# sayands/sgaligner

Hardware: AMD Instinct MI355X
Metric: subscan-pairs/sec (fwd+bwd) + node-match Hits@1 vs reference (higher is better)
Workload: dtype f32 (fp32 operands and fp32 accumulation throughout; the anchors x negatives loss sweeps multiply them as three exact bf16 planes, six bf16 MFMAs per product...

## Files before the change

sgaligner_amd/csrc/sweep3.hip:

```cpp
#include <type_traits>

#include "loss_math.h"

namespace {

typedef __bf16 bf16x8 __attribute__((ext_vector_type(8)));
typedef __bf16 bf16x2 __attribute__((ext_vector_type(2)));
typedef float f32x2 __attribute__((ext_vector_type(2)));
typedef unsigned int u32x4 __attribute__((ext_vector_type(4)));
typedef unsigned int u32x2 __attribute__((ext_vector_type(2)));
typedef short s16x4 __attribute__((ext_vector_type(4)));

constexpr int S3_DP = 104;
constexpr int S3_PLANE = 3 * 2 * 1024;
constexpr int S3_TAIL = 3 * S3_PLANE;
constexpr int S3_BLOCK = S3_TAIL + 2048;
constexpr int S3_NCH = S3_BLOCK / 1024;
constexpr int S3_ROWSLOTS = 3 * 12 + 4;

__device__ __forceinline__ void split3_pair(float v0, float v1, unsigned& h, unsigned& m, unsigned& l) {
    const bf16x2 H = __builtin_convertvector(f32x2{v0, v1}, bf16x2);
    const unsigned hu = __builtin_bit_cast(unsigned, H);
#ifdef S3_SPLIT_DOT2
    unsigned c0 = 0x0000BF80u, c1 = 0xBF800000u;
    asm("" : "+s"(c0), "+s"(c1));
    const bf16x2 n0 = __builtin_bit_cast(bf16x2, c0), n1 = __builtin_bit_cast(bf16x2, c1);
    const float r0 = __builtin_amdgcn_fdot2_f32_bf16(H, n0, v0, false);
    const float r1 = __builtin_amdgcn_fdot2_f32_bf16(H, n1, v1, false);
#else
    const float r0 = v0 - __builtin_bit_cast(float, hu << 16);
    const float r1 = v1 - __builtin_bit_cast(float, hu & 0xffff0000u);
#endif
    const bf16x2 Mi = __builtin_convertvector(f32x2{r0, r1}, bf16x2);
    const unsigned mu = __builtin_bit_cast(unsigned, Mi);
#ifdef S3_SPLIT_DOT2
    const float s0 = __builtin_amdgcn_fdot2_f32_bf16(Mi, n0, r0, false);
    const float s1 = __builtin_amdgcn_fdot2_f32_bf16(Mi, n1, r1, false);
#else
    const float s0 = r0 - __builtin_bit_cast(float, mu << 16);
    const float s1 = r1 - __builtin_bit_cast(float, mu & 0xffff0000u);
#endif
    const bf16x2 Lo = __builtin_convertvector(f32x2{s0, s1}, bf16x2);
    h = hu; m = mu; l = __builtin_bit_cast(unsigned, Lo);
}
__device__ __forceinline__ f32x4 mfma_b(u32x4 a, u32x4 b, f32x4 c) {
    return __builtin_amdgcn_mfma_f32_16x16x32_bf16(__builtin_bit_cast(bf16x8, a), __builtin_bit_cast(bf16x8, b), c, 0, 0, 0);
}
__device__ __forceinline__ u32x2 tr_read16(const unsigned char* p) {
    return __builtin_bit_cast(u32x2, __builtin_amdgcn_ds_read_tr16_b64_v4i16((__attribute__((address_space(3))) s16x4*)(p)));
}
__device__ __forceinline__ unsigned long long sreg64(unsigned long long v) {
    const unsigned lo = __builtin_amdgcn_readfirstlane((unsigned)v), hi = __builtin_amdgcn_readfirstlane((unsigned)(v >> 32));
    return ((unsigned long long)hi << 32) | lo;
}
template <int X, int END, int NR, bool VALU_ALL> __device__ __forceinline__ void sgb_seq() {
    if constexpr (X < END) {
        __builtin_amdgcn_sched_group_barrier(0x008, 1, 0);
        if constexpr (X < NR) __builtin_amdgcn_sched_group_barrier(0x100, 1, 0);
        if constexpr (VALU_ALL || X < 2) __builtin_amdgcn_sched_group_barrier(0x002, 2, 0);
        sgb_seq<X + 1, END, NR, VALU_ALL>();
    }
}
__host__ __device__ constexpr int s3_slot(int g, int i) { return 16 * g + (i ^ (12 * (g & 1))); }

struct TLayout { int nbA, nb1, nb2; };
__host__ __device__ inline TLayout make_tlayout(int A, int J1, int J2) { return TLayout{(A + 31) / 32, (J1 + 31) / 32, (J2 + 31) / 32}; }

constexpr int S3_STAT_BYTES = 2048;
constexpr int S3_DREAL = 100;

constexpr int S3_CS_BLOCKS = 256;
__global__ __launch_bounds__(128) void split3_colsum_kernel(const float* __restrict__ Z, int R, double* __restrict__ part) {
    const int c = threadIdx.x;
    const int per = (R + gridDim.x - 1) / gridDim.x, r0 = blockIdx.x * per, r1 = min(R, r0 + per);
    if (c >= S3_DP) return;
    double acc = 0.0;
    for (int r = r0; r < r1; ++r) acc += (double)Z[(size_t)r * S3_DP + c];
    part[(size_t)blockIdx.x * S3_DP + c] = acc;
}
__global__ __launch_bounds__(128) void split3_stats_kernel(const double* __restrict__ part, int nblocks, int R, float* __restrict__ stat) {
    __shared__ double sq[128];
    const int c = threadIdx.x;
    double cs = 0.0;
    if (c < S3_DP) for (int b = 0; b < nblocks; ++b) cs += part[(size_t)b * S3_DP + c];
    float zb = (c < S3_DREAL && R > 0) ? (float)(cs / (double)R) : 0.f;
    sq[c] = (double)zb * (double)zb;
    __syncthreads();
    __shared__ double tot;
    if (c == 0) {
        double t = 0.0;
        for (int i = 0; i < 128; ++i) t += sq[i];
        tot = t;
    }
    __syncthreads();
    const bool centre = tot >= 0.25;
    if (!centre) zb = 0.f;
    if (c < S3_DP) stat[c] = zb;
    if (c == 0) { stat[S3_DP] = centre ? (float)(0.5 * tot) : 0.f; stat[S3_DP + 1] = centre ? 1.f : 0.f; }
}

__global__ __launch_bounds__(256) void split3_tables_kernel(const float* __restrict__ Z, int A, int J1, int J2, unsigned char* __restrict__ Zb,
                                                            const float* __restrict__ stat, float* __restrict__ Zc) {
    __shared__ float tile[32 * S3_DP];
    __shared__ float zbar[S3_DP];
    const TLayout L = make_tlayout(A, J1, J2);
    int b = blockIdx.x, old0, len;
    if (b < L.nbA) { old0 = 0; len = A; }
    else if (b < 2 * L.nbA) { b -= L.nbA; old0 = A; len = A; }
    else if (b < 2 * L.nbA + L.nb1) { b -= 2 * L.nbA; old0 = 2 * A; len = J1; }
    else { b -= 2 * L.nbA + L.nb1; old0 = 2 * A + J1; len = J2; }
    const int nvalid = min(32, len - 32 * b);
    const float* src = Z + (size_t)(old0 + 32 * b) * S3_DP;
    if (threadIdx.x < S3_DP) zbar[threadIdx.x] = stat[threadIdx.x];
    __syncthreads();
    for (int e = threadIdx.x; e < 32 * S3_DP; e += 256) {
        const int r = e / S3_DP, c = e - r * S3_DP;
        tile[e] = (r < nvalid && c < S3_DREAL) ? src[e] - zbar[c] : 0.f;
        if (Zc && old0 < 2 * A && r < nvalid) Zc[(size_t)(old0 + 32 * b) * S3_DP + e] = c == S3_DREAL + 1 ? 1.f : tile[e];
    }
    __syncthreads();
    if (threadIdx.x < 32) {
        const int r = threadIdx.x;
        if (r < nvalid) {
            double a = 0.0;
            for (int c = 0; c < S3_DREAL; ++c) a += (double)zbar[c] * (double)tile[r * S3_DP + c];
            tile[r * S3_DP + S3_DREAL] = (float)(a + (double)stat[S3_DP]);
            tile[r * S3_DP + S3_DREAL + 1] = 1.f;
        }
    }
    __syncthreads();
    unsigned* out = reinterpret_cast<unsigned*>(Zb + (size_t)blockIdx.x * S3_BLOCK);
    for (int e = threadIdx.x; e < 3 * 2 * 64 * 4; e += 256) {
        const int p = e & 3, st = (e >> 2) & 63, jh = (e >> 8) & 1, q = e >> 9;
        const int g = st >> 4, i = (st & 15) ^ (12 * (g & 1));
        const int row = 8 * (i >> 2) + 4 * jh + (i & 3), col = 32 * q + 8 * g + 2 * p;
        unsigned h, m, l;
        split3_pair(tile[row * S3_DP + col], tile[row * S3_DP + col + 1], h, m, l);
        out[e] = h; out[S3_PLANE / 4 + e] = m; out[2 * S3_PLANE / 4 + e] = l;
    }
    for (int e = threadIdx.x; e < 2 * 64 * 4; e += 256) {
        const int p = e & 3, st = (e >> 2) & 63, jh = (e >> 8) & 1;
        const int g = st >> 4, i = (st & 15) ^ (12 * (g & 1));
        const int row = 8 * (i >> 2) + 4 * jh + (i & 3), col = 96 + 2 * p;
        unsigned h, m, l;
        split3_pair(tile[row * S3_DP + col], tile[row * S3_DP + col + 1], h, m, l);
        out[S3_TAIL / 4 + e] = g < 2 ? h : (g == 2 ? m : l);
    }
}


__global__ __launch_bounds__(256) void centre_tables_kernel(const float* __restrict__ Z, int R, const float* __restrict__ stat, float* __restrict__ Zc) {
    const int lane = threadIdx.x & 63, wpb = blockDim.x >> 6;
    for (int r = blockIdx.x * wpb + (threadIdx.x >> 6); r < R; r += gridDim.x * wpb) {
        const float* z = Z + (size_t)r * S3_DP;
        float* o = Zc + (size_t)r * S3_DP;
        double acc = 0.0;
        float v[2];
#pragma unroll
        for (int t = 0; t < 2; ++t) {
            const int d = lane + 64 * t;
            const float zb = d < S3_DREAL ? stat[d] : 0.f;
            v[t] = d < S3_DREAL ? z[d] - zb : 0.f;
            acc += (double)zb * (double)v[t];
        }
        acc = wave_sum_d(acc);
        o[lane] = v[0];
        const int d1 = lane + 64;
        if (d1 < S3_DP) o[d1] = d1 < S3_DREAL ? v[1] : (d1 == S3_DREAL ? (float)(acc + (double)stat[S3_DP]) : (d1 == S3_DREAL + 1 ? 1.f : 0.f));
    }
}

#ifdef S3_DBG_TIMING
__device__ unsigned long long g_s3_dbg[16];
#define S3_T(i) { const unsigned long long t_ = __builtin_readcyclecounter(); tacc[i] += t_ - tprev; tprev = t_; }
#else
#define S3_T(i)
#endif
struct TSeg { int blk0, jt_lo, jt_hi, old0, lo, hi, fam; };
struct TGroup { int own0, nown, own_old0, own_blk0, blk0, nsplit, nseg; TSeg seg[2]; };
struct TArgs {
    int M; const unsigned char* Zb[4]; int perm[4]; int ngroups; TGroup grp[4];
    float k0, k1, it0, it1, ka;
    const float* beta;
    double* sums;
    const double* gs;
    float* dZ[4];
    double* gamma;
};

template <int M, bool GRAD, int WV, int MG, bool GAM, bool LITE, bool FOLD>
__device__ __forceinline__ void sweep3_body(const TArgs& a, const int g) {
    static_assert(!LITE || !GRAD, "LITE: the forward sums only");
    static_assert(!FOLD || (GRAD && WV == 4), "FOLD: the one-wave-per-SIMD gradient sweep only");
    constexpr int NCT = 7;
    constexpr int WAVES = WV, THREADS = WAVES * 64;
    constexpr int OWN = WV * 16;
    constexpr int NCH = LITE ? S3_NCH - S3_PLANE / 1024 : S3_NCH;
    constexpr int KMAX = (NCH + WAVES - 1) / WAVES;
    constexpr int BUF = M * S3_BLOCK;
    constexpr bool PIPE = WV == 4;
#ifndef S3_OWN_IN_S
#define S3_OWN_IN_S 1
#endif
    constexpr bool OWN_IN_S = GRAD && PIPE && S3_OWN_IN_S;
#ifndef S3_SPREAD
#define S3_SPREAD 1
#endif
    constexpr bool SPREAD = OWN_IN_S && S3_SPREAD && !FOLD;
    extern __shared__ __attribute__((aligned(16))) unsigned char lds3[];

    const int tid = threadIdx.x, lane = tid & 63, wave = tid >> 6, g4 = lane >> 4, l15 = lane & 15;
    const TGroup& grp = a.grp[g];
    const int wg_in_grp = (int)blockIdx.x - grp.blk0;
    const int nsplit = grp.nsplit, n_ob = (grp.nown + OWN - 1) / OWN, n_units = n_ob * nsplit;
    const int unit = (wg_in_grp & 7) * ((n_units + 7) >> 3) + (wg_in_grp >> 3);
    if ((wg_in_grp >> 3) >= ((n_units + 7) >> 3) || unit >= n_units) return;
    const int split = unit / n_ob;
    const int own0 = grp.own0 + (unit - split * n_ob) * OWN;
    const int own_end = grp.own0 + grp.nown;
    const int wrow0 = own0 + wave * 16;
#ifdef S3_DBG_TIMING
    unsigned long long tacc[8] = {0, 0, 0, 0, 0, 0, 0, 0}, tprev = __builtin_readcyclecounter();
#endif

    u32x4 opl[M][3][3], otl[M][2];
    float beta[M];
    const bool iv = wrow0 + l15 < own_end;
    {
        const int my_i = wrow0 + l15;
        const int rel = (iv ? my_i : own0) - grp.own_old0;
        const int o = rel & 31, oi = 4 * (o >> 3) + (o & 3), ojh = (o >> 2) & 1;
        const size_t off = (size_t)(grp.own_blk0 + (rel >> 5)) * S3_BLOCK;
#pragma unroll
        for (int m = 0; m < M; ++m) {
            const unsigned char* base = a.Zb[m] + off;
#pragma unroll
            for (int p = 0; p < 3; ++p)
#pragma unroll
                for (int q = 0; q < 3; ++q) {
                    const int so = ((q * 2 + ojh) * 64 + s3_slot(g4, oi)) * 16;
                    opl[m][p][q] = iv ? *reinterpret_cast<const u32x4*>(base + p * S3_PLANE + so) : u32x4{0, 0, 0, 0};
                }
            u32x4 th = iv ? *reinterpret_cast<const u32x4*>(base + S3_TAIL + (ojh * 64 + s3_slot(0, oi)) * 16) : u32x4{0, 0, 0, 0};
            u32x4 tm = iv ? *reinterpret_cast<const u32x4*>(base + S3_TAIL + (ojh * 64 + s3_slot(2, oi)) * 16) : u32x4{0, 0, 0, 0};
            u32x4 tl = iv ? *reinterpret_cast<const u32x4*>(base + S3_TAIL + (ojh * 64 + s3_slot(3, oi)) * 16) : u32x4{0, 0, 0, 0};
            const float ksc = a.k1;
            auto rescale = [&](u32x4& ph, u32x4& pm, u32x4& pl) {
#pragma unroll
                for (int d = 0; d < 4; ++d) {
                    const float x0 = (__builtin_bit_cast(float, ph[d] << 16) + __builtin_bit_cast(float, pm[d] << 16)) + __builtin_bit_cast(float, pl[d] << 16);
                    const float x1 = (__builtin_bit_cast(float, ph[d] & 0xffff0000u) + __builtin_bit_cast(float, pm[d] & 0xffff0000u)) + __builtin_bit_cast(float, pl[d] & 0xffff0000u);
                    unsigned nh, nm, nl;
                    split3_pair(x0 * ksc, x1 * ksc, nh, nm, nl);
                    ph[d] = nh; pm[d] = nm; pl[d] = nl;
                }
            };
#pragma unroll
            for (int q = 0; q < 3; ++q) rescale(opl[m][0][q], opl[m][1][q], opl[m][2][q]);
            rescale(th, tm, tl);
            otl[m][0] = g4 == 1 ? tm : th;
            otl[m][1] = g4 == 0 ? tl : (g4 == 2 ? tm : u32x4{0, 0, 0, 0});
#pragma unroll
            for (int t = 0; t < 2; ++t)
                otl[m][t][2] = (otl[m][t][2] >> 16) | (otl[m][t][2] << 16);
        }
    }
#pragma unroll
    for (int m = 0; m < M; ++m) beta[m] = a.beta[a.perm[m]];

    constexpr int NSM = GRAD ? (FOLD ? 1 : MG) : 1;
    f32x4 gacc[GRAD ? MG : 1][NCT], gsm[NSM][NCT];
#pragma unroll
    for (int m = 0; m < (GRAD ? MG : 1); ++m)
#pragma unroll
        for (int ct = 0; ct < NCT; ++ct) gacc[m][ct] = f32x4{0.f, 0.f, 0.f, 0.f};
#pragma unroll
    for (int m = 0; m < NSM; ++m)
#pragma unroll
        for (int ct = 0; ct < NCT; ++ct) gsm[m][ct] = f32x4{0.f, 0.f, 0.f, 0.f};
    float gam[M];
#pragma unroll
    for (int m = 0; m < M; ++m) gam[m] = 0.f;

    const int wave_u = __builtin_amdgcn_readfirstlane(wave);
    const unsigned l16 = (threadIdx.x & 63u) * 16u;
    __amdgpu_buffer_rsrc_t rs[M];
    typedef __attribute__((address_space(3))) unsigned char* lds_ptr;
    constexpr bool LAST_ODD = KMAX * WAVES > NCH || (LITE && KMAX * WAVES > 2 * (S3_PLANE / 1024));
    unsigned crot[M], clast[M], trot[M], brot[M];
    unsigned tile_off = 0, buf_off = 0;
#pragma unroll
    for (int m = 0; m < M; ++m) {
        const int rot = (wave_u + m) & (WAVES - 1);
        int c = rot + (KMAX - 1) * WAVES;
        c = c >= NCH ? c - WAVES : c;
        if (LITE) c = c >= 2 * (S3_PLANE / 1024) ? c + S3_PLANE / 1024 : c;
        crot[m] = (unsigned)rot * 1024u; clast[m] = (unsigned)c * 1024u;
        trot[m] = 0; brot[m] = 0;
    }
    auto set_seg = [&](const TSeg& sgm) {
#pragma unroll
        for (int m = 0; m < M; ++m)
            rs[m] = __builtin_amdgcn_make_buffer_rsrc(const_cast<unsigned char*>(a.Zb[m]) + (size_t)sgm.blk0 * S3_BLOCK, (short)0,
                                                      (int)((unsigned)sgm.jt_hi * (unsigned)S3_BLOCK), 0x00020000);
    };
    auto set_tile = [&](int jt, unsigned char* buf) {
        tile_off = (unsigned)jt * (unsigned)S3_BLOCK;
        buf_off = (unsigned)(buf - lds3);
#pragma unroll
        for (int m = 0; m < M; ++m) {
            trot[m] = tile_off + crot[m]; brot[m] = buf_off + (unsigned)(m * S3_BLOCK) + crot[m];
            asm("" : "+s"(trot[m]), "+s"(brot[m]));
        }
    };
    auto issue_slots = [&](int f_lo, int f_hi) {
#ifdef S3_DBG_NODMA
        return;
#endif
#ifdef S3_DBG_DMA_WAVES
        unsigned dma_mask = S3_DBG_DMA_WAVES;
        asm volatile("" : "+s"(dma_mask));
        if (!((dma_mask >> wave_u) & 1u)) return;
#endif
#pragma unroll
        for (int f = f_lo; f < f_hi; ++f) {
            if (f >= M * KMAX) break;
            const int m = f / KMAX, k = f % KMAX;
            unsigned so, lo;
            if (LAST_ODD && k == KMAX - 1) { so = tile_off + clast[m]; lo = buf_off + (unsigned)(m * S3_BLOCK) + clast[m]; }
            else { so = trot[m] + (unsigned)(k * WAVES * 1024); lo = brot[m] + (unsigned)(k * WAVES * 1024); }
            __builtin_amdgcn_raw_ptr_buffer_load_lds(rs[m], (lds_ptr)lds3 + lo, 16, l16, so, 0, 0);
        }
    };
    auto issue = [&](int jt, unsigned char* buf) { set_tile(jt, buf); issue_slots(0, M * KMAX); };

    const int aoff = s3_slot(g4, l15) * 16;
    const int tr_io = 4 * g4 + (l15 >> 2), tr_cs = l15 & 3;
    const int tr_main = s3_slot(tr_cs >> 1, tr_io) * 16 + (tr_cs & 1) * 8;
    const int tr_tail = S3_TAIL + tr_io * 16 + (tr_cs & 1) * 8;
    const int tr_tail_l = S3_TAIL + (48 + (tr_io ^ 12)) * 16 + (tr_cs & 1) * 8;

#pragma unroll 1
    for (int sg = 0; sg < 2; ++sg) {
        if (sg >= grp.nseg) break;
        const TSeg seg = grp.seg[sg];
        set_seg(seg);
        float c0[M + 1], c1[M + 1];
#pragma unroll
        for (int m = 0; m <= M; ++m) {
            const int mo = m < M ? a.perm[m] : M;
            c0[m] = GRAD ? (float)(a.gs[mo * 8 + seg.fam * 2 + 0] * (double)a.it0) : 0.f;
            c1[m] = GRAD ? (float)(a.gs[mo * 8 + seg.fam * 2 + 1] * (double)a.it1) : 0.f;
        }
        const float ka = a.ka;
        double dsum[M + 1][2];
#pragma unroll
        for (int m = 0; m <= M; ++m) { dsum[m][0] = 0.0; dsum[m][1] = 0.0; }
        float pl0[LITE ? M + 1 : 1], pl1[LITE ? M + 1 : 1];
#pragma unroll
        for (int m = 0; m < (LITE ? M + 1 : 1); ++m) { pl0[m] = 0.f; pl1[m] = 0.f; }

        __syncthreads();
        if (seg.jt_lo + split < seg.jt_hi) issue(seg.jt_lo + split, lds3);
        int it = 0;
#pragma unroll 1
        for (int jt = seg.jt_lo + split; jt < seg.jt_hi; jt += nsplit, ++it) {
            unsigned char* buf = lds3 + (it & 1) * BUF;
            const int j0 = seg.old0 + 32 * jt;
            S3_T(5)
            __syncthreads();
            S3_T(0)
            const int next_jt = jt + nsplit < seg.jt_hi ? jt + nsplit : jt;
            unsigned char* next_buf = lds3 + ((it + 1) & 1) * BUF;
            set_tile(next_jt, next_buf);
            S3_T(1)
            if (GRAD) {
                const int vlo = max(seg.lo - j0, 0), vhi = min(seg.hi - j0, 32);
                if (vlo > 0 || vhi < 32) {
                    for (int x = tid; x < M * 32 * S3_ROWSLOTS; x += THREADS) {
                        const int pc = x % S3_ROWSLOTS, w = (x / S3_ROWSLOTS) % 32, m = x / (S3_ROWSLOTS * 32);
                        if (w >= vlo && w < vhi) continue;
                        const int wjh = (w >> 2) & 1, wi = 4 * (w >> 3) + (w & 3);
                        unsigned char* base = buf + m * S3_BLOCK;
                        if (pc < 36) {
                            const int pl = pc / 12, q = (pc % 12) >> 2, gq = pc & 3;
                            *reinterpret_cast<u32x4*>(base + pl * S3_PLANE + ((q * 2 + wjh) * 64 + s3_slot(gq, wi)) * 16) = u32x4{0, 0, 0, 0};
                        } else {
                            const int gq = pc - 36;
                            *reinterpret_cast<u32x4*>(base + S3_TAIL + (wjh * 64 + s3_slot(gq, wi)) * 16) = u32x4{0, 0, 0, 0};
                        }
                    }
                    __syncthreads();
                }
            }

            f32x4 sacc[M][2];
            float own[M][2][4];
            float cj[2][4];
            auto substep_wait = [&](int ss) {
                if (ss > 0) { __builtin_amdgcn_s_waitcnt(0xc07f); __builtin_amdgcn_sched_barrier(0); }
            };
            constexpr int NSET = PIPE ? 2 : 1;
            u32x4 at[NSET], ap[NSET][3][3];
            auto ld_one = [&](int ss, int idx) {
                const int e = ss % NSET;
                const unsigned char* ar = buf + (SPREAD ? ss % M : ss >> 1) * S3_BLOCK + (SPREAD ? ss / M : ss & 1) * 1024 + aoff;
                if (idx < 1) at[e] = *reinterpret_cast<const u32x4*>(ar + S3_TAIL);
                else ap[e][2 - (idx - 1) / 3][(idx - 1) % 3] = *reinterpret_cast<const u32x4*>(ar + (2 - (idx - 1) / 3) * S3_PLANE + ((idx - 1) % 3) * 2048);
            };
            auto ld_set = [&](int ss) {
#pragma unroll
                for (int idx = 0; idx < 10; ++idx) if (!(LITE && idx >= 1 && idx <= 3)) ld_one(ss, idx);
            };
            if (PIPE) {
                ld_set(0);
                __builtin_amdgcn_s_waitcnt(0xc07f);
                __builtin_amdgcn_sched_barrier(0);
            }
            if constexpr (SPREAD) {
                constexpr int NDS = 2 * M - 2, PER = (M * KMAX + NDS - 1) / NDS;
                constexpr int PA[6] = {2, 1, 1, 0, 0, 0}, PB[6] = {0, 1, 0, 2, 1, 0};
                f32x4 accp[2][2];
                float ot0 = 0.f, ot1 = 0.f, sjt = 0.f, ce0 = 0.f, ce1 = 0.f;
                auto own_step = [&](int mm, int hh, int r, int k) {
                    const float sv = sacc[mm][hh][r];
                    if (k == 0) ot0 = fexp2(sv * ka);
                    else if (k == 1) ot1 = fexp2(sv);
                    else own[mm][hh][r] = fmaf(c0[mm], ot0, c1[mm] * ot1);
                };
                auto cj_step = [&](int hh, int r, int k) {
                    if (k == 0) {
                        sjt = 0.f;
#pragma unroll
                        for (int mm = 0; mm < M; ++mm) sjt = fmaf(beta[mm], sacc[mm][hh][r], sjt);
                    } else if (k == 1) ce0 = fexp2(sjt * ka);
                    else if (k == 2) ce1 = fexp2(sjt);
                    else cj[hh][r] = c0[M] * ce0 + c1[M] * ce1;
                };
#pragma unroll
                for (int ss = 0; ss < 2 * M; ++ss) {
                    const int m = ss % M, jh = ss / M, e = ss % NSET, pa = ss & 1;
                    const int pm = ss > 0 ? (ss - 1) % M : 0, pjh = ss > 0 ? (ss - 1) / M : 0;
                    accp[pa][0] = f32x4{0.f, 0.f, 0.f, 0.f}; accp[pa][1] = f32x4{0.f, 0.f, 0.f, 0.f};
                    substep_wait(ss);
#pragma unroll
                    for (int x = 0; x < 20; ++x) {
                        if (x == 0) accp[pa][0] = mfma_b(at[e], otl[m][1], accp[pa][0]);
                        else if (x == 1) accp[pa][1] = mfma_b(at[e], otl[m][0], accp[pa][1]);
                        else accp[pa][x & 1] = mfma_b(ap[e][PA[(x - 2) / 3]][(x - 2) % 3], opl[m][PB[(x - 2) / 3]][(x - 2) % 3], accp[pa][x & 1]);
                        __builtin_amdgcn_sched_barrier(0);
                        if (ss + 1 < 2 * M && x < 10) ld_one(ss + 1, x);
                        if (ss < NDS && (x % 3) == 1 && (x / 3) < PER) issue_slots(ss * PER + (x / 3), ss * PER + (x / 3) + 1);
                        if (ss > 0) {
                            if (x == 0) { sacc[pm][pjh][0] = accp[pa ^ 1][0][0] + accp[pa ^ 1][1][0]; sacc[pm][pjh][1] = accp[pa ^ 1][0][1] + accp[pa ^ 1][1][1]; }
                            if (x == 2) { sacc[pm][pjh][2] = accp[pa ^ 1][0][2] + accp[pa ^ 1][1][2]; sacc[pm][pjh][3] = accp[pa ^ 1][0][3] + accp[pa ^ 1][1][3]; }
                            if (pm < MG) {
                                constexpr int G0[4] = {3, 8, 12, 16}, G1[4] = {5, 9, 14, 17}, G2[4] = {6, 11, 15, 18};
#pragma unroll
                                for (int r = 0; r < 4; ++r) {
                                    if (x == G0[r]) own_step(pm, pjh, r, 0);
                                    if (x == G1[r]) own_step(pm, pjh, r, 1);
                                    if (x == G2[r]) own_step(pm, pjh, r, 2);
                                }
                            }
                        }
                        if (ss >= NDS) {
                            const int q = (x == 19 ? 5 : (x % 3) == 1 && x <= 13 ? x / 3 : -1);
                            if (q >= 0) {
                                const int qq = (ss - NDS) * 6 + q, r = qq / 3, k = qq % 3;
                                if (k == 0) { if (r > 0) cj_step(0, r - 1, 3); cj_step(0, r, 0); }
                                else cj_step(0, r, k);
                            }
                        }
                        __builtin_amdgcn_sched_barrier(0);
                    }
                }
#pragma unroll
                for (int r = 0; r < 4; ++r) sacc[M - 1][1][r] = accp[(2 * M - 1) & 1][0][r] + accp[(2 * M - 1) & 1][1][r];
                cj_step(0, 3, 3);
            } else {
#pragma unroll
            for (int ss = 0; ss < 2 * M; ++ss) {
                const int m = ss >> 1, jh = ss & 1, e = ss % NSET;
                if (!PIPE) ld_set(ss);
                if (PIPE) substep_wait(ss);
                constexpr int NDS = GRAD ? (2 * M - 2) : 2 * M, PER = (M * KMAX + NDS - 1) / NDS;
                f32x4 acc2[2] = {f32x4{0.f, 0.f, 0.f, 0.f}, f32x4{0.f, 0.f, 0.f, 0.f}};
                float ownt[2] = {0.f, 0.f};
                constexpr int PA[6] = {2, 1, 1, 0, 0, 0}, PB[6] = {0, 1, 0, 2, 1, 0};
#pragma unroll
                for (int x = 0; x < 20; ++x) {
                    const bool skip = LITE && x >= 2 && (PA[(x - 2) / 3] == 2 || PB[(x - 2) / 3] == 2 || (PA[(x - 2) / 3] == 1 && PB[(x - 2) / 3] == 1));
                    if (skip) {}
                    else if (x == 0) acc2[0] = mfma_b(at[e], otl[m][1], acc2[0]);
                    else if (x == 1) acc2[1] = mfma_b(at[e], otl[m][0], acc2[1]);
                    else acc2[x & 1] = mfma_b(ap[e][PA[(x - 2) / 3]][(x - 2) % 3], opl[m][PB[(x - 2) / 3]][(x - 2) % 3], acc2[x & 1]);
                    if (PIPE) {
                        __builtin_amdgcn_sched_barrier(0);
                        if (ss + 1 < 2 * M && x < 10 && !(LITE && x >= 1 && x <= 3)) ld_one(ss + 1, x);
                        if (ss < NDS && (x % 3) == 1 && (x / 3) < PER) issue_slots(ss * PER + (x / 3), ss * PER + (x / 3) + 1);
                        if (OWN_IN_S && m > 0 && m - 1 < MG && x >= 11 && x < 19) {
                            const int r = (x - 11) >> 1;
                            const float sv = sacc[m - 1][jh][r];
                            if (((x - 11) & 1) == 0) {
                                ownt[0] = fexp2(sv * ka);
                                ownt[1] = fexp2(sv);
                            } else {
                                own[m - 1][jh][r] = fmaf(c0[m - 1], ownt[0], c1[m - 1] * ownt[1]);
                            }
                        }
                        __builtin_amdgcn_sched_barrier(0);
                    } else if (x == 1 && ss < NDS) {
                        issue_slots(ss * PER, (ss + 1) * PER);
                    }
                }
#pragma unroll
                for (int r = 0; r < 4; ++r) sacc[m][jh][r] = acc2[0][r] + acc2[1][r];
            }
            }

            S3_T(2)
            if (!GRAD) {
                float p0[M + 1], p1[M + 1];
#pragma unroll
                for (int m = 0; m <= M; ++m) { p0[m] = LITE ? pl0[LITE ? m : 0] : 0.f; p1[m] = LITE ? pl1[LITE ? m : 0] : 0.f; }
                auto sums_tile = [&](auto masked_c) {
                    constexpr bool MASKED = decltype(masked_c)::value;
#pragma unroll
                    for (int jh = 0; jh < 2; ++jh)
#pragma unroll
                        for (int r = 0; r < 4; ++r) {
                            const int row = j0 + 8 * g4 + 4 * jh + r;
                            const float okf = (!MASKED || (iv && row >= seg.lo && row < seg.hi)) ? 1.f : 0.f;
                            float sj = 0.f;
#pragma unroll
                            for (int m = 0; m < M; ++m) {
                                const float sv = sacc[m][jh][r];
                                sj = fmaf(beta[m], sv, sj);
                                p0[m] = MASKED ? fmaf(okf, fexp2(sv * ka), p0[m]) : p0[m] + fexp2(sv * ka);
                                p1[m] = MASKED ? fmaf(okf, fexp2(sv), p1[m]) : p1[m] + fexp2(sv);
                            }
                            p0[M] = MASKED ? fmaf(okf, fexp2(sj * ka), p0[M]) : p0[M] + fexp2(sj * ka);
                            p1[M] = MASKED ? fmaf(okf, fexp2(sj), p1[M]) : p1[M] + fexp2(sj);
                        }
                };
                if (j0 >= seg.lo && j0 + 32 <= seg.hi && own0 + OWN <= own_end) sums_tile(std::false_type{}); else sums_tile(std::true_type{});
                if (!LITE || (it & 3) == 3) {
#pragma unroll
                    for (int m = 0; m <= M; ++m) { dsum[m][0] += (double)p0[m]; dsum[m][1] += (double)p1[m]; }
#pragma unroll
                    for (int m = 0; m < (LITE ? M + 1 : 1); ++m) { pl0[m] = 0.f; pl1[m] = 0.f; }
                } else {
#pragma unroll
                    for (int m = 0; m < (LITE ? M + 1 : 1); ++m) { pl0[m] = p0[m]; pl1[m] = p1[m]; }
                }
            } else {
                constexpr int BD = PIPE ? 4 : 1;
                u32x4 bp[BD][3];
                auto ld_b = [&](int k) {
                    const int m = k / NCT, ct = k % NCT, par = k % BD;
                    const unsigned char* pb = buf + m * S3_BLOCK;
#pragma unroll
                    for (int p = 0; p < 3; ++p) {
                        const unsigned char* ph = ct < 6 ? pb + p * S3_PLANE + tr_main + (ct >> 1) * 2048 + (ct & 1) * 512
                                                         : pb + (p == 2 ? tr_tail_l : tr_tail + (p == 1 ? 512 : 0));
                        const u32x2 x0 = tr_read16(ph), x1 = tr_read16(ph + 1024);
                        bp[par][p] = u32x4{x0[0], x0[1], x1[0], x1[1]};
                    }
                };
                auto own_last = [&]() {
#pragma unroll
                    for (int r = 0; r < 4; ++r) {
                        const float sv = sacc[M - 1][1][r];
                        own[M - 1][1][r] = fmaf(c0[M - 1], fexp2(sv * ka), c1[M - 1] * fexp2(sv));
                    }
                };
#pragma unroll
                for (int m = SPREAD ? M : OWN_IN_S ? M - 1 : 0; m < MG; ++m)
#pragma unroll
                    for (int jh = 0; jh < 2; ++jh)
#pragma unroll
                        for (int r = 0; r < 4; ++r) {
                            const float sv = sacc[m][jh][r];
#ifdef S3_DBG_NOEPI
                            own[m][jh][r] = sv;
#else
                            own[m][jh][r] = fmaf(c0[m], fexp2(sv * ka), c1[m] * fexp2(sv));
#endif
                        }
#pragma unroll
                for (int jh = SPREAD ? 1 : 0; jh < 2; ++jh)
#pragma unroll
                    for (int r = 0; r < 4; ++r) {
                        float sj = 0.f;
#pragma unroll
                        for (int m = 0; m < M; ++m) sj = fmaf(beta[m], sacc[m][jh][r], sj);
#ifdef S3_DBG_NOEPI
                        cj[jh][r] = sj;
#else
                        cj[jh][r] = c0[M] * fexp2(sj * ka) + c1[M] * fexp2(sj);
#endif
                    }
                auto gamma_acc = [&]() {
#pragma unroll
                    for (int m = 0; m < M; ++m) {
#pragma unroll
                        for (int jh = 0; jh < 2; ++jh)
#pragma unroll
                            for (int r = 0; r < 4; ++r) gam[m] = fmaf(cj[jh][r], sacc[m][jh][r], gam[m]);
                    }
                };
                if ((!PIPE || FOLD) && GAM) gamma_acc();
                S3_T(3)
                u32x4 ch[2], cm[2], cl[2];
                auto planes = [&](int m) {
#pragma unroll
                    for (int p = 0; p < 4; ++p) {
                        const int jh = p >> 1, r = (p & 1) * 2;
#ifdef S3_DBG_NOEPI
                        const float v0 = own[m][jh][r] + cj[jh][r], v1 = own[m][jh][r + 1] + cj[jh][r + 1];
#else
                        const float v0 = fmaf(beta[m], cj[jh][r], own[m][jh][r]), v1 = fmaf(beta[m], cj[jh][r + 1], own[m][jh][r + 1]);
#endif
                        unsigned h_, m_, l_;
                        split3_pair(v0, v1, h_, m_, l_);
                        ch[m & 1][p] = h_; cm[m & 1][p] = m_; cl[m & 1][p] = l_;
                    }
                };
                planes(0);
                auto step_small = [&](int m, int ct, int par, int i) {
                    const int e = m & 1;
                    const u32x4 ca = i == 0 ? cl[e] : (i == 1 || i == 4) ? ch[e] : cm[e];
                    const int pb_ = i == 0 ? 0 : i == 1 ? 2 : i == 2 ? 1 : i == 3 ? 0 : 1;
                    const int sm = (GRAD && !FOLD) ? m : 0;
                    gsm[sm][ct] = mfma_b(ca, bp[par][pb_], (FOLD && i == 0) ? f32x4{0.f, 0.f, 0.f, 0.f} : gsm[sm][ct]);
                };
                auto fold_group = [&](int gq) {
                    const int m = gq >> 2, ct0 = (gq & 3) * 2, n = (gq & 3) == 3 ? 1 : 2;
#pragma unroll
                    for (int j = 0; j < n; ++j)
#pragma unroll
                        for (int r = 0; r < 4; ++r) gacc[GRAD ? m : 0][ct0 + j][r] += gsm[0][ct0 + j][r];
                };
                if (!PIPE) {
#pragma unroll
                    for (int m = 0; m < MG; ++m) {
                        if (m > 0) planes(m);
#pragma unroll
                        for (int ct = 0; ct < NCT; ++ct) {
                            ld_b(NCT * m + ct);
#pragma unroll
                            for (int i = 0; i < 5; ++i) step_small(m, ct, 0, i);
                            gacc[GRAD ? m : 0][ct] = mfma_b(ch[m & 1], bp[0][0], gacc[GRAD ? m : 0][ct]);
                        }
                    }
                } else {
                    __builtin_amdgcn_sched_barrier(0);
                    ld_b(0); ld_b(1);
                    __builtin_amdgcn_sched_barrier(0);
#pragma unroll
                    for (int g4i = 0; g4i < 4 * MG; ++g4i) {
                        const int m = g4i >> 2, ct0 = (g4i & 3) * 2, n = (g4i & 3) == 3 ? 1 : 2, k0_ = NCT * m + ct0;
                        if (SPREAD && g4i == 0 && M - 1 < MG && M > 1) own_last();
                        if ((g4i & 3) == 0 && m + 1 < MG) planes(m + 1);
                        if (GAM && !FOLD && g4i == (MG > 1 ? 4 : 0)) gamma_acc();
                        if (FOLD && g4i >= 2) fold_group(g4i - 2);
                        const int kn = k0_ + n;
                        const int nn = kn >= NCT * MG ? 0 : ((kn % NCT) == 6 ? 1 : 2);
#pragma unroll
                        for (int j = 0; j < nn; ++j) ld_b(kn + j);
                        if (n == 2) {
#pragma unroll
                            for (int i = 0; i < 5; ++i) { step_small(m, ct0, k0_ % BD, i); step_small(m, ct0 + 1, (k0_ + 1) % BD, i); }
                            gacc[GRAD ? m : 0][ct0] = mfma_b(ch[m & 1], bp[k0_ % BD][0], gacc[GRAD ? m : 0][ct0]);
                            gacc[GRAD ? m : 0][ct0 + 1] = mfma_b(ch[m & 1], bp[(k0_ + 1) % BD][0], gacc[GRAD ? m : 0][ct0 + 1]);
                        } else {
                            step_small(m, ct0, k0_ % BD, 0);
                            gacc[GRAD ? m : 0][ct0] = mfma_b(ch[m & 1], bp[k0_ % BD][0], gacc[GRAD ? m : 0][ct0]);
#pragma unroll
                            for (int i = 1; i < 5; ++i) step_small(m, ct0, k0_ % BD, i);
                        }
                        if (FOLD) {
                            if (n == 2) { if (nn == 2) sgb_seq<0, 12, 12, true>(); else if (nn == 1) sgb_seq<0, 12, 6, true>(); else sgb_seq<0, 12, 0, true>(); }
                            else { if (nn == 2) sgb_seq<0, 6, 12, false>(); else if (nn == 1) sgb_seq<0, 6, 6, false>(); else sgb_seq<0, 6, 0, false>(); }
                        } else {
#pragma unroll
                        for (int x = 0; x < 6 * n; ++x) {
                            __builtin_amdgcn_sched_group_barrier(0x008, 1, 0);
                            if (x < 6 * nn) __builtin_amdgcn_sched_group_barrier(0x100, 1, 0);
                            if (n == 2 || x < 2) __builtin_amdgcn_sched_group_barrier(0x002, 2, 0);
                        }
                        }
                        if ((g4i & 3) == 3) __builtin_amdgcn_sched_barrier(0);
                    }
                    if (FOLD) { fold_group(4 * MG - 2); fold_group(4 * MG - 1); }
                }
                S3_T(4)
            }
        }
        if (!GRAD) {
#pragma unroll
            for (int m = 0; m <= M; ++m)
#pragma unroll
                for (int tt = 0; tt < 2; ++tt) {
                    if (LITE) dsum[m][tt] += (double)(tt ? pl1[LITE ? m : 0] : pl0[LITE ? m : 0]);
                    const double v = wave_sum_d(dsum[m][tt]);
                    if (lane == 0 && v != 0.0) atomicAdd(a.sums + (M + 1) * 8 * (1 + my_slot()) + m * 8 + seg.fam * 2 + tt, v);
                }
        }
    }
#ifdef S3_DBG_TIMING
    if (lane == 0) for (int i = 0; i < 8; ++i) atomicAdd(&g_s3_dbg[(GRAD ? 8 : 0) + i], tacc[i]);
#endif
    if (GRAD) {
#pragma unroll
        for (int m = 0; m < MG; ++m) {
            float* dz = a.dZ[m];
#pragma unroll
            for (int ct = 0; ct < NCT; ++ct) if (!FOLD) gacc[GRAD ? m : 0][ct] += gsm[(GRAD && !FOLD) ? m : 0][ct];
#pragma unroll
            for (int ct = 0; ct < NCT; ++ct) {
                const int d = ct * 16 + l15;
                if (d < S3_DREAL || d == S3_DREAL + 1) {
#pragma unroll
                    for (int r = 0; r < 4; ++r) {
                        const int i = wrow0 + 4 * g4 + r;
                        if (i < own_end) atomicAdd(dz + (size_t)i * S3_DP + d, gacc[GRAD ? m : 0][ct][r]);
                    }
                }
            }
        }
        if (GAM && g < 2) {
#pragma unroll
            for (int m = 0; m < M; ++m) {
                const float v = wave_sum(gam[m]) / a.k1;
                if (lane == 0 && v != 0.f) atomicAdd(a.gamma + M * (1 + my_slot()) + a.perm[m], (double)v);
            }
        }
    }
}

template <int M, bool GRAD, int WV, int MG = M, bool GAM = true, bool LITE = false, bool FOLD = false>
__global__ __launch_bounds__(WV * 64, WV == 8 ? 2 : 1) void sweep3_kernel(TArgs a) {
    int g = 0;
#pragma unroll
    for (int i = 1; i < 4; ++i) if (i < a.ngroups && (int)blockIdx.x >= a.grp[i].blk0) g = i;
#ifndef S3_GAM_ALL
    if constexpr (GRAD && GAM) {
        if (g >= 2) { sweep3_body<M, GRAD, WV, MG, false, LITE, FOLD>(a, g); return; }
    }
#endif
    sweep3_body<M, GRAD, WV, MG, GAM, LITE, FOLD>(a, g);
}

struct SProd { const float* S; int ld, tn, own_seg, own0, nown, oth_seg, oth0, noth, blk0, nsplit; };
struct SArgs { const unsigned char* Zb; float* dZ; const float* zero; int A, nbA, n; SProd p[4]; };

__global__ __launch_bounds__(256, 2) void stash3_kernel(SArgs a) {
    constexpr int NCT = 7, WAVES = 4, RW = 2, OWN = WAVES * RW * 16;
    constexpr int KMAX = (S3_NCH + WAVES - 1) / WAVES;
    extern __shared__ __attribute__((aligned(16))) unsigned char lds3[];
    const int tid = threadIdx.x, lane = tid & 63, wave = tid >> 6, g4 = lane >> 4, l15 = lane & 15;
    int pi = 0;
#pragma unroll
    for (int i = 1; i < 4; ++i) if (i < a.n && (int)blockIdx.x >= a.p[i].blk0) pi = i;
    const SProd& P = a.p[pi];
    const float* const PS = P.S;
    const float* const zero_word = a.zero;
    const int Pld = P.ld, Ptn = P.tn, Pnown = P.nown, Poth0 = P.oth0, Pnoth = P.noth;
    const int w_in = (int)blockIdx.x - P.blk0;
    const int n_ob = (P.nown + OWN - 1) / OWN;
    if (w_in >= n_ob * P.nsplit) return;
    const int split = w_in / n_ob, ob = w_in - split * n_ob;
    const int orow0 = ob * OWN + wave * (RW * 16) + l15;
    const int t_lo = P.oth0 >> 5, t_hi = (P.oth0 + P.noth + 31) >> 5;
    const int per = (t_hi - t_lo + P.nsplit - 1) / P.nsplit;
    const int jt0 = t_lo + split * per, jt1 = min(t_hi, jt0 + per);
    if (jt0 >= jt1) return;
    const int oblk0 = P.oth_seg ? a.nbA : 0;

    const int wave_u = __builtin_amdgcn_readfirstlane(wave);
    unsigned l16 = threadIdx.x;
    asm volatile("" : "+v"(l16));
    l16 = (l16 & 63u) * 16u;
    auto issue = [&](int blk, unsigned char* buf) {
        const unsigned long long tb = sreg64(reinterpret_cast<unsigned long long>(a.Zb) + (unsigned long long)blk * S3_BLOCK);
#pragma unroll
        for (int k = 0; k < KMAX; ++k) {
            int c = wave_u + k * WAVES;
            if ((k + 1) * WAVES > S3_NCH) c = c >= S3_NCH ? c - WAVES : c;
            __builtin_amdgcn_global_load_lds((const __attribute__((address_space(1))) void*)(reinterpret_cast<const unsigned char*>(tb + (unsigned)(c * 1024)) + l16),
                                             (__attribute__((address_space(3))) void*)(buf + c * 1024), 16, 0, 0);
        }
    };
    auto load_c = [&](int jt, int rs, float (&c)[8]) {
        const int orow = orow0 + 16 * rs;
        const bool ov = orow < Pnown;
        const int r0 = 32 * jt + 8 * g4 - Poth0;
        if (!Ptn && (Pld & 3) == 0 && (Poth0 & 3) == 0 && ov && r0 >= 0 && r0 + 8 <= Pnoth) {
            const f32x4* q = reinterpret_cast<const f32x4*>(PS + (size_t)orow * Pld + r0);
            const f32x4 u = q[0], v = q[1];
            c[0] = u[0]; c[1] = u[1]; c[2] = u[2]; c[3] = u[3]; c[4] = v[0]; c[5] = v[1]; c[6] = v[2]; c[7] = v[3];
        } else {
            const float* base = PS + (Ptn ? (size_t)orow : (size_t)orow * Pld);
            const int stride = Ptn ? Pld : 1;
            const unsigned lim = ov ? (unsigned)Pnoth : 0u;
#pragma unroll
            for (int k = 0; k < 8; ++k) {
                const int t = r0 + k;
                const bool ok = (unsigned)t < lim;
                const float* q = ok ? base + (size_t)t * stride : zero_word;
                c[k] = *q;
            }
        }
    };

    f32x4 gacc[RW][NCT], gsm[RW][NCT];
#pragma unroll
    for (int rs = 0; rs < RW; ++rs)
#pragma unroll
        for (int ct = 0; ct < NCT; ++ct) { gacc[rs][ct] = f32x4{0.f, 0.f, 0.f, 0.f}; gsm[rs][ct] = f32x4{0.f, 0.f, 0.f, 0.f}; }
    const int tr_io = 4 * g4 + (l15 >> 2), tr_cs = l15 & 3;
    const int tr_main = s3_slot(tr_cs >> 1, tr_io) * 16 + (tr_cs & 1) * 8;
    const int tr_tail = S3_TAIL + tr_io * 16 + (tr_cs & 1) * 8;
    const int tr_tail_l = S3_TAIL + (48 + (tr_io ^ 12)) * 16 + (tr_cs & 1) * 8;

    float c0[RW][8], c1[RW][8];
#pragma unroll
    for (int rs = 0; rs < RW; ++rs) {
        load_c(jt0, rs, c0[rs]);
        if (jt0 + 1 < jt1) load_c(jt0 + 1, rs, c1[rs]);
    }
    issue(oblk0 + jt0, lds3);
    int it = 0;
    auto step = [&](int jt, float (&cc)[RW][8]) {
        unsigned char* buf = lds3 + (it & 1) * S3_BLOCK;
        __syncthreads();
        issue(oblk0 + (jt + 1 < jt1 ? jt + 1 : jt), lds3 + ((it + 1) & 1) * S3_BLOCK);
        u32x4 ch[RW], cm[RW], cl[RW];
#pragma unroll
        for (int rs = 0; rs < RW; ++rs)
#pragma unroll
            for (int p = 0; p < 4; ++p) {
                unsigned h_, m_, l_;
                split3_pair(cc[rs][2 * p], cc[rs][2 * p + 1], h_, m_, l_);
                ch[rs][p] = h_; cm[rs][p] = m_; cl[rs][p] = l_;
            }
        if (jt + 2 < jt1) {
#pragma unroll
            for (int rs = 0; rs < RW; ++rs) load_c(jt + 2, rs, cc[rs]);
        }
#pragma unroll
        for (int ct = 0; ct < NCT; ++ct) {
            u32x4 bp[3];
#pragma unroll
            for (int p = 0; p < 3; ++p) {
                const unsigned char* ph = ct < 6 ? buf + p * S3_PLANE + tr_main + (ct >> 1) * 2048 + (ct & 1) * 512
                                                 : buf + (p == 2 ? tr_tail_l : tr_tail + (p == 1 ? 512 : 0));
                const u32x2 x0 = tr_read16(ph), x1 = tr_read16(ph + 1024);
                bp[p] = u32x4{x0[0], x0[1], x1[0], x1[1]};
            }
#pragma unroll
            for (int rs = 0; rs < RW; ++rs) gsm[rs][ct] = mfma_b(cl[rs], bp[0], gsm[rs][ct]);
#pragma unroll
            for (int rs = 0; rs < RW; ++rs) gsm[rs][ct] = mfma_b(ch[rs], bp[2], gsm[rs][ct]);
#pragma unroll
            for (int rs = 0; rs < RW; ++rs) gsm[rs][ct] = mfma_b(cm[rs], bp[1], gsm[rs][ct]);
#pragma unroll
            for (int rs = 0; rs < RW; ++rs) gsm[rs][ct] = mfma_b(cm[rs], bp[0], gsm[rs][ct]);
#pragma unroll
            for (int rs = 0; rs < RW; ++rs) gsm[rs][ct] = mfma_b(ch[rs], bp[1], gsm[rs][ct]);
#pragma unroll
            for (int rs = 0; rs < RW; ++rs) gacc[rs][ct] = mfma_b(ch[rs], bp[0], gacc[rs][ct]);
        }
        ++it;
    };
#pragma unroll 1
    for (int jt = jt0; jt < jt1; jt += 2) {
        step(jt, c0);
        if (jt + 1 < jt1) step(jt + 1, c1);
    }
    float* dz = a.dZ + (size_t)(P.own_seg ? a.A : 0) * S3_DP;
#pragma unroll
    for (int rs = 0; rs < RW; ++rs)
#pragma unroll
        for (int ct = 0; ct < NCT; ++ct) {
            const int d = ct * 16 + l15;
            if (d < S3_DREAL || d == S3_DREAL + 1) {
#pragma unroll
                for (int r = 0; r < 4; ++r) {
                    const int o = ob * OWN + wave * (RW * 16) + 16 * rs + 4 * g4 + r;
                    if (o < P.nown) atomicAdd(dz + (size_t)(P.own0 + o) * S3_DP + d, gacc[rs][ct][r] + gsm[rs][ct][r]);
                }
            }
        }
}

int fill_t(TArgs& a, const void* const* Zb, int M, const float* beta, int A, int J1, int J2, float tau0, float tau1, bool grad,
           int a_lo, int a_hi, int own_rows, const char* who) {
    if (M < 2 || M > 4) { sga_set_error("%s: M=%d (the three-plane bf16 sweeps are built for 2, 3 or 4 modality tables)", who, M); return SGA_ERR_ARG; }
    if (a_lo < 0 || a_hi > A || a_lo > a_hi) { sga_set_error("%s: anchor shard [%d,%d) outside [0,%d]", who, a_lo, a_hi, A); return SGA_ERR_ARG; }
    a.M = M;
    const TLayout L = make_tlayout(A, J1, J2);
    for (int m = 0; m < M; ++m) {
        if (!Zb[m]) { sga_set_error("%s: null table", who); return SGA_ERR_ARG; }
        a.Zb[m] = static_cast<const unsigned char*>(Zb[m]);
        a.perm[m] = m;
    }
    a.beta = beta; a.k0 = LOG2E / tau0; a.k1 = LOG2E / tau1; a.it0 = 1.f / tau0; a.it1 = 1.f / tau1; a.ka = a.k0 / a.k1;
    const int ns = a_hi - a_lo;
    const int bx1 = 0, bx2 = L.nbA, bn1 = 2 * L.nbA, bn2 = 2 * L.nbA + L.nb1;
    const int ox1 = 0, ox2 = A, on1 = 2 * A, on2 = 2 * A + J1;
    const TSeg N1a{bn1, 0, L.nb1, on1, on1, on1 + J1, 0}, N2a{bn2, 0, L.nb2, on2, on2, on2 + J2, 1};
    const TSeg N2b{bn2, 0, L.nb2, on2, on2, on2 + J2, 2}, N1b{bn1, 0, L.nb1, on1, on1, on1 + J1, 3};
    int g = 0;
    auto add = [&](int own0, int nown, int own_old0, int own_blk0, TSeg s0, TSeg s1) {
        if (nown <= 0) return;
        TGroup& G = a.grp[g++];
        G.own0 = own0; G.nown = nown; G.own_old0 = own_old0; G.own_blk0 = own_blk0; G.nseg = 2; G.seg[0] = s0; G.seg[1] = s1; G.nsplit = 1; G.blk0 = 0;
    };
    add(ox1 + a_lo, ns, ox1, bx1, N1a, N2a);
    add(ox2 + a_lo, ns, ox2, bx2, N2b, N1b);
    if (grad) {
        const int jl = a_lo / 32, jh = (a_hi + 31) / 32;
        const TSeg X1f0{bx1, jl, jh, ox1, ox1 + a_lo, ox1 + a_hi, 0}, X2f3{bx2, jl, jh, ox2, ox2 + a_lo, ox2 + a_hi, 3};
        const TSeg X1f1{bx1, jl, jh, ox1, ox1 + a_lo, ox1 + a_hi, 1}, X2f2{bx2, jl, jh, ox2, ox2 + a_lo, ox2 + a_hi, 2};
        add(on1, J1, on1, bn1, X1f0, X2f3);
        add(on2, J2, on2, bn2, X1f1, X2f2);
    }
    a.ngroups = g;
    for (int i = 0; i < g; ++i)
        for (int sg = 0; sg < a.grp[i].nseg; ++sg)
            if ((long long)a.grp[i].seg[sg].jt_hi * S3_BLOCK >= (1LL << 32)) {
                sga_set_error("%s: a segment of %d 32-row blocks exceeds the 4 GiB a copy descriptor spans", who, a.grp[i].seg[sg].jt_hi);
                return SGA_ERR_ARG;
            }
    int nwg = 0;
    for (int i = 0; i < g; ++i) {
        TGroup& G = a.grp[i];
        int steps = 0;
        for (int sg = 0; sg < G.nseg; ++sg) steps += G.seg[sg].jt_hi - G.seg[sg].jt_lo;
        const long n_ob_g = (G.nown + own_rows - 1) / own_rows;
        const long want = (long)steps * n_ob_g / (12L * sga_num_cus());
        const int unit_steps = want < 160 ? 160 : want > 640 ? 640 : (int)want;
        int nsp = (steps + unit_steps - 1) / unit_steps;
        if (nsp > steps) nsp = steps;
        if (nsp < 1) nsp = 1;
        G.nsplit = nsp;
        G.blk0 = nwg;
        nwg += (((G.nown + own_rows - 1) / own_rows) * nsp + 7) / 8 * 8;
    }
    return -nwg;
}

#ifndef S3_WV_SUMS
#define S3_WV_SUMS 8
#endif
#ifndef S3_WV_GRAD3
#define S3_WV_GRAD3 4
#endif
#ifndef S3_WV_GRAD2
#define S3_WV_GRAD2 4
#endif
template <int M, bool GRAD> constexpr int s3_wv() { return M == 4 ? 4 : GRAD ? (M == 3 ? S3_WV_GRAD3 : S3_WV_GRAD2) : S3_WV_SUMS; }

template <int M, bool GRAD, int MG = M, bool GAM = true, bool LITE = false, bool FOLD = false>
// ... 214 lines not shown
```

Baseline: 984.4.

## Interleave paired S-stream MFMA chains with double-buffered loads and epilogue

Adds a paired S-stream mode that runs two independent MFMA accumulation chains at once (both halves of a column tile) and interleaves them with the next pair's LDS loads, slot copies and the exp2 owner/column epilogue work. The goal is to hide MFMA dependency latency and LDS latency by giving the scheduler two independent accumulators and by prefetching two operand sets ahead. The mode is on by default except for a few configurations (grad with M=2, forward M=4 non-lite, forward WV=8 M=3). In exchange it uses more VGPRs for the extra operand set and accumulators, and it relies on hand-tuned waitcnt values that can hurt occupancy or correctness if they are wrong.

```diff
diff --git a/sgaligner_amd/csrc/sweep3.hip b/sgaligner_amd/csrc/sweep3.hip
--- a/sgaligner_amd/csrc/sweep3.hip
+++ b/sgaligner_amd/csrc/sweep3.hip
@@ -188,6 +188,22 @@
     double* gamma;
 };
 
+#ifndef S3_PAIR
+#define S3_PAIR 1
+#endif
+template <int M, int PER> struct S3PairGaps {
+    int slot[M][40];
+    constexpr S3PairGaps() : slot{} {
+        for (int p = 0; p < M; ++p) {
+            int n = 0;
+            for (int P = 0; P < 40; ++P) {
+                const bool copy = p < M - 1 && P % (20 / PER) == 1 && P / (20 / PER) < 2 * PER;
+                slot[p][P] = (P >= 3 && !copy) ? n++ : -1;
+            }
+        }
+    }
+};
+
 template <int M, bool GRAD, int WV, int MG, bool GAM, bool LITE, bool FOLD>
 __device__ __forceinline__ void sweep3_body(const TArgs& a, const int g) {
     static_assert(!LITE || !GRAD, "LITE: the forward sums only");
@@ -207,6 +223,9 @@
 #define S3_SPREAD 1
 #endif
     constexpr bool SPREAD = OWN_IN_S && S3_SPREAD && !FOLD;
+    constexpr bool PAIR_FITS = !(!GRAD && WV == 8 && M == 3 && !LITE);
+    constexpr bool PAIR_DEFAULT = !(GRAD && M == 2) && !(!GRAD && M == 4 && !LITE);
+    constexpr bool PAIR = PAIR_FITS && (S3_PAIR == 2 || (S3_PAIR == 1 && PAIR_DEFAULT));
     extern __shared__ __attribute__((aligned(16))) unsigned char lds3[];
 
     const int tid = threadIdx.x, lane = tid & 63, wave = tid >> 6, g4 = lane >> 4, l15 = lane & 15;
@@ -400,7 +419,7 @@
             auto substep_wait = [&](int ss) {
                 if (ss > 0) { __builtin_amdgcn_s_waitcnt(0xc07f); __builtin_amdgcn_sched_barrier(0); }
             };
-            constexpr int NSET = PIPE ? 2 : 1;
+            constexpr int NSET = (PIPE || PAIR) ? 2 : 1;
             u32x4 at[NSET], ap[NSET][3][3];
             auto ld_one = [&](int ss, int idx) {
                 const int e = ss % NSET;
@@ -414,10 +433,93 @@
             };
             if (PIPE) {
                 ld_set(0);
+                if (PAIR) ld_set(1);
                 __builtin_amdgcn_s_waitcnt(0xc07f);
                 __builtin_amdgcn_sched_barrier(0);
             }
-            if constexpr (SPREAD) {
+            auto lgkm_wait = [&](int n) {
+                if (n == 0) __builtin_amdgcn_s_waitcnt(0xc07f);
+                else if (n == 6) __builtin_amdgcn_s_waitcnt(0xc67f);
+                else if (n == 8) __builtin_amdgcn_s_waitcnt(0xc87f);
+                else __builtin_amdgcn_s_waitcnt(0xce7f);
+                __builtin_amdgcn_sched_barrier(0);
+            };
+            if constexpr (SPREAD && PAIR) {
+                constexpr int NDS = 2 * M - 2, PER = (M * KMAX + NDS - 1) / NDS, CS = 20 / PER;
+                static_assert(2 * PER * CS <= 40 && (M - 1) * 2 * PER >= M * KMAX, "paired S stream: the copies' gaps");
+                constexpr int PA[6] = {2, 1, 1, 0, 0, 0}, PB[6] = {0, 1, 0, 2, 1, 0};
+                constexpr S3PairGaps<M, PER> GAPS{};
+                f32x4 accq[2][2];
+                float ot0 = 0.f, ot1 = 0.f, sjt = 0.f, ce0 = 0.f, ce1 = 0.f;
+                auto own_step = [&](int ss, int r, int k) {
+                    const int mm = ss % M, hh = ss / M;
+                    if (mm >= MG) return;
+                    const float sv = sacc[mm][hh][r];
+                    if (k == 0) ot0 = fexp2(sv * ka);
+                    else if (k == 1) ot1 = fexp2(sv);
+                    else own[mm][hh][r] = fmaf(c0[mm], ot0, c1[mm] * ot1);
+                };
+                auto cj_step = [&](int hh, int r, int k) {
+                    if (k == 0) {
+                        sjt = 0.f;
+#pragma unroll
+                        for (int mm = 0; mm < M; ++mm) sjt = fmaf(beta[mm], sacc[mm][hh][r], sjt);
+                    } else if (k == 1) ce0 = fexp2(sjt * ka);
+                    else if (k == 2) ce1 = fexp2(sjt);
+                    else cj[hh][r] = c0[M] * ce0 + c1[M] * ce1;
+                };
+                auto read_s = [&](int ss, const f32x4& acc) {
+#pragma unroll
+                    for (int r = 0; r < 4; ++r) {
+                        float v = acc[r];
+                        asm volatile("" : "+v"(v));
+                        sacc[ss % M][ss / M][r] = v;
+                    }
+                };
+#pragma unroll
+                for (int p = 0; p < M; ++p) {
+                    const int pp = p & 1;
+                    const bool nxt = p + 1 < M;
+                    accq[pp][0] = f32x4{0.f, 0.f, 0.f, 0.f}; accq[pp][1] = f32x4{0.f, 0.f, 0.f, 0.f};
+                    if (p > 0) lgkm_wait(6);
+#pragma unroll
+                    for (int P = 0; P < 40; ++P) {
+                        const int x = P >> 1, s = P & 1, m = (2 * p + s) % M;
+                        if (x == 0) accq[pp][s] = mfma_b(at[s], otl[m][1], accq[pp][s]);
+                        else if (x == 1) accq[pp][s] = mfma_b(at[s], otl[m][0], accq[pp][s]);
+                        else accq[pp][s] = mfma_b(ap[s][PA[(x - 2) / 3]][(x - 2) % 3], opl[m][PB[(x - 2) / 3]][(x - 2) % 3], accq[pp][s]);
+                        __builtin_amdgcn_sched_barrier(0);
+                        if (nxt) {
+                            const int sn = 2 * p + 2 + s;
+                            if (P >= 2 && P < 4) ld_one(sn, 0);
+                            else if (P >= 4 && P < 10) ld_one(sn, 1 + (P - 4) / 2);
+                            else if (P >= 16 && P < 22) ld_one(sn, 4 + (P - 16) / 2);
+                            else if (P >= 34) ld_one(sn, 7 + (P - 34) / 2);
+                        }
+                        if (p < M - 1 && (P % CS) == 1 && P / CS < 2 * PER) issue_slots(p * 2 * PER + P / CS, p * 2 * PER + P / CS + 1);
+                        if (p > 0) {
+                            if (P == 0) read_s(2 * p - 2, accq[pp ^ 1][0]);
+                            if (P == 2) read_s(2 * p - 1, accq[pp ^ 1][1]);
+                            const int fs = GAPS.slot[p][P];
+                            if (fs >= 0) {
+                                const int t = nxt ? fs : (fs % 3 < 2 ? 2 * (fs / 3) + fs % 3 : -1);
+                                const int qq = (!nxt && fs % 3 == 2) ? fs / 3 : -1;
+                                if (t >= 0 && t < 24) own_step(2 * p - 2 + ((t / 3) & 1), t / 6, t % 3);
+                                if (qq >= 0 && qq < 12) {
+                                    const int r = qq / 3, k = qq % 3;
+                                    if (k == 0) { if (r > 0) cj_step(0, r - 1, 3); cj_step(0, r, 0); }
+                                    else cj_step(0, r, k);
+                                }
+                            }
+                            if (P == 21) lgkm_wait(nxt ? 14 : 0);
+                        }
+                        __builtin_amdgcn_sched_barrier(0);
+                    }
+                }
+                read_s(2 * M - 2, accq[(M - 1) & 1][0]);
+                read_s(2 * M - 1, accq[(M - 1) & 1][1]);
+                cj_step(0, 3, 3);
+            } else if constexpr (SPREAD) {
                 constexpr int NDS = 2 * M - 2, PER = (M * KMAX + NDS - 1) / NDS;
                 constexpr int PA[6] = {2, 1, 1, 0, 0, 0}, PB[6] = {0, 1, 0, 2, 1, 0};
                 f32x4 accp[2][2];
@@ -478,6 +580,54 @@
 #pragma unroll
                 for (int r = 0; r < 4; ++r) sacc[M - 1][1][r] = accp[(2 * M - 1) & 1][0][r] + accp[(2 * M - 1) & 1][1][r];
                 cj_step(0, 3, 3);
+            } else if constexpr (PAIR) {
+                constexpr int NDS = GRAD ? (2 * M - 2) : 2 * M, PER = (M * KMAX + NDS - 1) / NDS, CS = 20 / PER;
+                static_assert(!PIPE || (2 * PER * CS <= 40 && (NDS / 2) * 2 * PER >= M * KMAX), "paired S stream: the copies' gaps");
+                constexpr int PA[6] = {2, 1, 1, 0, 0, 0}, PB[6] = {0, 1, 0, 2, 1, 0};
+#pragma unroll
+                for (int m = 0; m < M; ++m) {
+                    const bool nxt = m + 1 < M;
+                    if (!PIPE) { ld_set(2 * m); ld_set(2 * m + 1); }
+                    if (PIPE && m > 0) lgkm_wait(6);
+                    f32x4 accq[2] = {f32x4{0.f, 0.f, 0.f, 0.f}, f32x4{0.f, 0.f, 0.f, 0.f}};
+                    float ownt[2] = {0.f, 0.f};
+#pragma unroll
+                    for (int P = 0; P < 40; ++P) {
+                        const int x = P >> 1, s = P & 1;
+                        const bool skip = LITE && x >= 2 && (PA[(x - 2) / 3] == 2 || PB[(x - 2) / 3] == 2 || (PA[(x - 2) / 3] == 1 && PB[(x - 2) / 3] == 1));
+                        if (skip) {}
+                        else if (x == 0) accq[s] = mfma_b(at[s], otl[m][1], accq[s]);
+                        else if (x == 1) accq[s] = mfma_b(at[s], otl[m][0], accq[s]);
+                        else accq[s] = mfma_b(ap[s][PA[(x - 2) / 3]][(x - 2) % 3], opl[m][PB[(x - 2) / 3]][(x - 2) % 3], accq[s]);
+                        if (PIPE) {
+                            __builtin_amdgcn_sched_barrier(0);
+                            if (nxt) {
+                                const int sn = 2 * m + 2 + s;
+                                if (P >= 2 && P < 4) ld_one(sn, 0);
+                                else if (P >= 4 && P < 10) { if (!LITE) ld_one(sn, 1 + (P - 4) / 2); }
+                                else if (P >= 16 && P < 22) ld_one(sn, 4 + (P - 16) / 2);
+                                else if (P >= 34) ld_one(sn, 7 + (P - 34) / 2);
+                            }
+                            if (m < NDS / 2 && (P % CS) == 1 && P / CS < 2 * PER) issue_slots(m * 2 * PER + P / CS, m * 2 * PER + P / CS + 1);
+                            if (OWN_IN_S && m > 0 && m - 1 < MG && P >= 22 && P < 38) {
+                                const int r8 = (P - 22) >> 1;
+                                const float sv = sacc[m - 1][r8 >> 2][r8 & 3];
+                                if (((P - 22) & 1) == 0) {
+                                    ownt[0] = fexp2(sv * ka);
+                                    ownt[1] = fexp2(sv);
+                                } else {
+                                    own[m - 1][r8 >> 2][r8 & 3] = fmaf(c0[m - 1], ownt[0], c1[m - 1] * ownt[1]);
+                                }
+                            }
+                            if (m > 0 && P == 21) lgkm_wait(nxt ? (LITE ? 8 : 14) : 0);
+                            __builtin_amdgcn_sched_barrier(0);
+                        } else if (P == 1 && m < NDS / 2) {
+                            issue_slots(2 * m * PER, (2 * m + 2) * PER);
+                        }
+                    }
+#pragma unroll
+                    for (int r = 0; r < 4; ++r) { sacc[m][0][r] = accq[0][r]; sacc[m][1][r] = accq[1][r]; }
+                }
             } else {
 #pragma unroll
             for (int ss = 0; ss < 2 * M; ++ss) {
@@ -568,13 +718,19 @@
                         bp[par][p] = u32x4{x0[0], x0[1], x1[0], x1[1]};
                     }
                 };
-                auto own_last = [&]() {
+                constexpr int OWN_LAST0 = (SPREAD && PAIR) ? (M > 2 ? M - 2 : 1) : M - 1;
+                auto own_late = [&](int mm) {
 #pragma unroll
                     for (int r = 0; r < 4; ++r) {
-                        const float sv = sacc[M - 1][1][r];
-                        own[M - 1][1][r] = fmaf(c0[M - 1], fexp2(sv * ka), c1[M - 1] * fexp2(sv));
+                        const float sv = sacc[mm][1][r];
+                        own[mm][1][r] = fmaf(c0[mm], fexp2(sv * ka), c1[mm] * fexp2(sv));
                     }
                 };
+                auto own_last = [&]() {
+#pragma unroll
+                    for (int mm = OWN_LAST0; mm < M; ++mm) if (mm < MG) own_late(mm);
+                };
+                if (SPREAD && PAIR && M == 2) own_late(0);
 #pragma unroll
                 for (int m = SPREAD ? M : OWN_IN_S ? M - 1 : 0; m < MG; ++m)
 #pragma unroll
@@ -661,7 +817,7 @@
 #pragma unroll
                     for (int g4i = 0; g4i < 4 * MG; ++g4i) {
                         const int m = g4i >> 2, ct0 = (g4i & 3) * 2, n = (g4i & 3) == 3 ? 1 : 2, k0_ = NCT * m + ct0;
-                        if (SPREAD && g4i == 0 && M - 1 < MG && M > 1) own_last();
+                        if (SPREAD && g4i == 0 && OWN_LAST0 < MG && M > 1) own_last();
                         if ((g4i & 3) == 0 && m + 1 < MG) planes(m + 1);
                         if (GAM && !FOLD && g4i == (MG > 1 ? 4 : 0)) gamma_acc();
                         if (FOLD && g4i >= 2) fold_group(g4i - 2);
```

After: 995.5 (median of 6 runs). 1.01x the previous value.
